# OvO1111/JointImageGeneration

Hardware: AMD Instinct MI355X
Metric: sampled voxels/sec @50 DDIM steps, 128^3 mask + 512^2x256 CT (higher is better)
Workload: dtype bf16; 1 GPU; C5 full GuideGen volume per GPU: CCDM 128^3 K=14 250 steps -> LDM 256 slices x (cond-encode + 50 DDIM @4x64x64 + AE decode 512^2); volumes_per_gpu=1, ccdm_steps=250, ddim_steps=50, slices=256, parallelism=replicas x1 (one volume per GPU, no collective), weights=random-init (seed recipe)

## Files before the change

include/guidegen_hip.h:

```cpp
#ifndef GUIDEGEN_HIP_H
#define GUIDEGEN_HIP_H

#include <stdint.h>

#ifdef __cplusplus
extern "C" {
#endif

typedef enum {
    GG_OK = 0,
    GG_ERR_BAD_SHAPE = -1,
    GG_ERR_BAD_DTYPE = -2,
    GG_ERR_UNSUPPORTED = -3,
    GG_ERR_WORKSPACE_TOO_SMALL = -4,
    GG_ERR_HIP = -5
} gg_status;

typedef enum { GG_BF16 = 0, GG_F32 = 1 } gg_dtype;

const char *gg_last_error(void);
int gg_version(void);

typedef struct {
    int32_t N, D, H, W;
// ... 30 lines not shown
    int32_t pro_c_logical;
    const int64_t *pro_acc1;
    const int64_t *pro_acc2;
    const float *pro_gamma;
    const float *pro_beta;
    float pro_eps;
    int32_t skip_C1, skip_C2;
    int32_t reserved_tail;
    const void *skip_src1;
    const void *skip_src2;
    const void *skip_weight;
    const int32_t *post_xt;
    int32_t *post_labels_out;
    const float *post_scalars;
    const float *post_E;
    uint64_t post_philox_seed;
    const int64_t *post_philox_offset_dev;
    void *post_onehot_out;
    int64_t post_onehot_stride;
    int32_t post_draw;
    int32_t reserved_tail2;
    const uint64_t *post_philox_seeds;
    int64_t post_rows_per_sample;
} gg_conv_desc;

int64_t gg_conv_packed_weight_bytes(int32_t Cout, int32_t Cin_pad, int32_t ntaps);
int gg_conv_pack_weight(const float *w_f32, int32_t Cout, int32_t Cin, int32_t Cin_pad, int32_t ntaps,
                        void *packed_bf16, void *stream);
int64_t gg_conv_workspace_bytes(const gg_conv_desc *desc);
int gg_conv_fuses_prologue(const gg_conv_desc *desc);
int gg_conv_fuses_posterior(const gg_conv_desc *desc);
int gg_conv_runs_halo_tile(const gg_conv_desc *desc);
int gg_conv_runs_tile(const gg_conv_desc *desc);
int gg_conv_runs_halo_split(const gg_conv_desc *desc);
int gg_conv_runs_tile_s2(const gg_conv_desc *desc);
int gg_conv_emits_stats(const gg_conv_desc *desc);
int gg_conv_prologue_from_acc(const gg_conv_desc *desc);
int gg_conv_fuses_skip(const gg_conv_desc *desc);
int gg_conv_fuses_ddim(const gg_conv_desc *desc);
int gg_conv_forward(const gg_conv_desc *desc, void *stream);

int64_t gg_groupnorm_workspace_bytes(int32_t N, int64_t S, int32_t C);
int gg_groupnorm_stats(const void *src1, int32_t C1, const void *src2, int32_t C2, int32_t N, int64_t S,
                       int32_t C_logical, const float *gamma, const float *beta, float eps,
                       float *scale_out, float *shift_out, void *workspace, int64_t workspace_bytes, void *stream);
int gg_groupnorm_apply(const void *src1, int32_t C1, const void *src2, int32_t C2, int32_t N, int64_t S,
                       const float *scale, const float *shift, int32_t act, void *out, void *stream);
int gg_groupnorm_fused_supported(int64_t S, int32_t C1, int32_t C2, int32_t C_logical);
int gg_groupnorm_fused(const void *src1, int32_t C1, const void *src2, int32_t C2, int32_t N, int64_t S, int32_t C_logical,
                       const float *gamma, const float *beta, float eps, int32_t act, void *out, void *stream);
int gg_groupnorm_apply_acc(const void *src1, int32_t C1, const int64_t *acc1, const void *src2, int32_t C2, const int64_t *acc2,
                           int32_t N, int64_t S, int32_t C_logical, const float *gamma, const float *beta, float eps,
                           int32_t act, void *out, void *stream);

int gg_groupnorm_scale_shift_acc(const int64_t *acc1, int32_t stripes1, int32_t C1, const int64_t *acc2, int32_t stripes2, int32_t C2,
                                 int32_t N, int64_t S, int32_t C_logical, const float *gamma, const float *beta, float eps,
                                 float *scale_out, float *shift_out, void *stream);

int gg_resample2x(const void *src, int32_t dtype, int32_t N, int32_t D, int32_t H, int32_t W, int32_t C_pad, int32_t C_logical,
                  int32_t resample_d, int32_t mode, const float *scale, const float *shift, int32_t act, void *dst, void *stream);
int gg_film_fold(float *scale, float *shift, int32_t coef_stride, int32_t N, int32_t C, const float *film, int64_t film_stride, void *stream);

typedef struct {
    int32_t N, heads, head_dim;
    int32_t Tq, Tkv;
    int64_t ldq, hsq, ldk, hsk, ldv, hsv, ldo, hso;
    float scale;
    int32_t reserved;
    const void *q, *k, *v;
    void *out;
    void *workspace;
    int64_t workspace_bytes;
} gg_attention_desc;
int gg_attention_forward(const gg_attention_desc *desc, void *stream);
int64_t gg_attention_workspace_bytes(const gg_attention_desc *desc);
int gg_attention_plan(const gg_attention_desc *desc, int32_t plan[4]);
int gg_attention_forward_kvlen(const gg_attention_desc *desc, const int32_t *kv_len, void *stream);

// ... 158 lines not shown
```

jointimagegeneration_amd/csrc/gg_conv.h:

```cpp
#pragma once
#include "gg_common.h"

struct ConvParams {
    int N, D, H, W, C1, C2, Cout, Cout_pad;
    int kd, kh, kw, stride, pad, upsample;
    int Do, Ho, Wo, out_dtype, prologue_act;
    int path_hint;
    int nchunk1, nchunk, ntaps;
    long long M;
    long long bias_stride;
    const bf16_t *src1, *src2, *weight, *residual;
    const float *bias, *gn_scale, *gn_shift;
    void *out;
    float *ws;
    int splitk;
    long long *gn_acc;
    float *ddim_x, *ddim_pred_x0;
    const float *ddim_scalars;
    bf16_t *ddim_unet_in;
    long long ddim_unet_in_stride;
    unsigned mg_osp, mg_ohw, mg_wo;
    int epi_geglu;
    const long long *pro_acc1, *pro_acc2;
    const float *pro_gamma, *pro_beta;
// ... 41 lines not shown

__device__ __forceinline__ float gg_row16_sum(float x)
{
    x += __builtin_bit_cast(float, __builtin_amdgcn_mov_dpp(__builtin_bit_cast(int, x), 0xB1, 0xF, 0xF, true));
    x += __builtin_bit_cast(float, __builtin_amdgcn_mov_dpp(__builtin_bit_cast(int, x), 0x4E, 0xF, 0xF, true));
    x += __builtin_bit_cast(float, __builtin_amdgcn_mov_dpp(__builtin_bit_cast(int, x), 0x141, 0xF, 0xF, true));
    x += __builtin_bit_cast(float, __builtin_amdgcn_mov_dpp(__builtin_bit_cast(int, x), 0x140, 0xF, 0xF, true));
    return x;
}

__device__ __forceinline__ f32x4 gg_conv_epi_value(f32x4 acc, bool has_bias, f32x4 bv, bool has_res, bf16x4 res, int co, int Cout)
{
    f32x4 v = acc;
    if (has_bias) v += bv;
    if (has_res) {
#pragma unroll
        for (int j = 0; j < 4; ++j) v[j] += (float)res[j];
    }
#pragma unroll
    for (int j = 0; j < 4; ++j)
        if (co + j >= Cout) v[j] = 0.f;
    return v;
}
__device__ __forceinline__ bf16x4 gg_conv_epi_bf16(f32x4 v)
{
    bf16x4 ob;
#pragma unroll
    for (int j = 0; j < 4; ++j) ob[j] = (bf16_t)v[j];
    return ob;
}

int gg_conv_tile_try(const ConvParams &p, hipStream_t stream);
int gg_conv_tile_family(const ConvParams &p);
bool gg_conv_tile_s2_family(const ConvParams &p);
int gg_conv_tile_s2_launch(const ConvParams &p, hipStream_t stream);
bool gg_conv_halo_split_box_fits(const ConvParams &p);
int gg_conv_halo_split_launch(const ConvParams &p, hipStream_t stream);
```

jointimagegeneration_amd/csrc/gg_conv.hip:

```cpp
#include "gg_norm.h"
#include <stdlib.h>

template <int NT, int PF, int PRO>
__global__ __launch_bounds__(256) void conv_gather_kernel(const ConvParams p)
{
    constexpr int BM = 128;
    constexpr int XBYTES = BM * 64;
    constexpr int WBYTES = NT * 32 * 64;
    constexpr int STAGE = XBYTES + WBYTES;
    constexpr int WITER = (NT * 128 + 255) / 256;
    __shared__ __attribute__((aligned(16))) char smem[2 * STAGE];

    const int tid = threadIdx.x;
    const int lane = tid & 63;
    const int wave = tid >> 6;
    const long long m0 = (long long)blockIdx.x * BM;
    const int g0 = blockIdx.y * NT;

    const int xq = tid & 3;
    int bn[2], bd[2], bh[2], bw[2];
    bool rv[2];
    const bf16_t *rb1[2], *rb2[2];
    const unsigned osp = (unsigned)(p.Do * p.Ho * p.Wo);
    const unsigned ohw = (unsigned)(p.Ho * p.Wo);
// ... 767 lines not shown
    if (!GG_HALO_SPLIT || !gg_hint_is_production(p.path_hint) || p.path_hint == GG_CONV_HINT_NO_HALO_SPLIT) return 0;
    if (p.kd != 3 || p.kh != 3 || p.kw != 3 || p.stride != 1 || p.pad != 1 || p.upsample || p.prologue_act) return 0;
    if (d->epilogue_geglu || d->post_xt || d->ddim_x || d->skip_C1) return 0;
    if (halo_try_dry(p) || box_try_dry(p) || !gg_conv_halo_split_box_fits(p)) return 0;
    if (gg_conv_tiny_plan(p.M, p.Cout_pad, p.ntaps * p.nchunk, p.prologue_act) || plan_gather5(p.M, p.C1, p.C2, p.Cout_pad, p.ntaps)) return 0;
    const GatherPlan pl = plan_gather(p.M, p.Cout_pad, p.ntaps * p.nchunk);
    return (pl.NT == 1 && pl.splitk >= 2 && p.nchunk % pl.splitk == 0) ? pl.splitk : 0;
}

extern "C" int gg_conv_runs_halo_split(const gg_conv_desc *d)
{
    if (!desc_channels_ok(d)) return 0;
    ConvParams p;
    fill_params(d, p);
    return plan_halo_split(d, p);
}

static bool plan_tile_s2(const gg_conv_desc *d, const ConvParams &p)
{
    if (!gg_conv_tile_s2_family(p) || halo_try_dry(p) || box_try_dry(p)) return false;
    if (p.path_hint == GG_CONV_HINT_TILE_S2) return true;
    if (gg_conv_tiny_plan(p.M, p.Cout_pad, p.ntaps * p.nchunk, p.prologue_act) || plan_gather5(p.M, p.C1, p.C2, p.Cout_pad, p.ntaps)) return false;
    return plan_gather(p.M, p.Cout_pad, p.ntaps * p.nchunk).splitk == 1;
}

extern "C" int gg_conv_runs_tile_s2(const gg_conv_desc *d)
{
    if (!desc_channels_ok(d)) return 0;
    ConvParams p;
    fill_params(d, p);
    return plan_tile_s2(d, p) ? 1 : 0;
}

#ifdef GG_EXP_WPREFETCH
__global__ __launch_bounds__(256) void exp_wprefetch_kernel(const u32x4 *w, long long n16, unsigned *sink)
{
    unsigned a = 0;
    if (n16 <= (3 << 20) / 16 * 1) {
        for (long long i = (long long)(blockIdx.x >> 3) * 256 + threadIdx.x; i < n16; i += 32 * 256) { const u32x4 v = w[i]; a ^= v[0] ^ v[1] ^ v[2] ^ v[3]; }
    } else
    for (long long i = (long long)blockIdx.x * 256 + threadIdx.x; i < n16; i += 256 * 256) { const u32x4 v = w[i]; a ^= v[0] ^ v[1] ^ v[2] ^ v[3]; }
    if (a == 0x12345679u) sink[0] = a;
}
#endif
extern "C" int gg_conv_forward(const gg_conv_desc *d, void *stream_)
{
    hipStream_t stream = (hipStream_t)stream_;
    if (!d) GG_FAIL(GG_ERR_BAD_SHAPE, "conv: null desc");
    if (d->C1 <= 0 || d->C1 % 32 || d->C2 % 32 || d->C2 < 0) GG_FAIL(GG_ERR_BAD_SHAPE, "conv: C1/C2 must be multiples of 32 (got %d, %d)", d->C1, d->C2);
    if (d->Cout_pad % 32 || d->Cout > d->Cout_pad || d->Cout <= 0) GG_FAIL(GG_ERR_BAD_SHAPE, "conv: bad Cout/Cout_pad %d/%d", d->Cout, d->Cout_pad);
    auto okk = [](int k) { return k == 1 || k == 3; };
    if (!okk(d->kd) || !okk(d->kh) || !okk(d->kw)) GG_FAIL(GG_ERR_UNSUPPORTED, "conv: kernel extent must be 1 or 3");
    if (d->stride != 1 && d->stride != 2) GG_FAIL(GG_ERR_UNSUPPORTED, "conv: stride must be 1 or 2");
    if (d->upsample && d->stride != 1) GG_FAIL(GG_ERR_UNSUPPORTED, "conv: upsample with stride");
    if (d->out_dtype != GG_BF16 && d->out_dtype != GG_F32) GG_FAIL(GG_ERR_BAD_DTYPE, "conv: out dtype");
    if (!d->src1 || !d->weight || (!d->out && !d->post_xt) || (d->C2 && !d->src2)) GG_FAIL(GG_ERR_BAD_SHAPE, "conv: null pointer");
    if (d->post_xt) {
        if (!gg_conv_fuses_posterior(d)) GG_FAIL(GG_ERR_UNSUPPORTED, "conv: this shape cannot run the fused CCDM reverse step (gg_conv_fuses_posterior)");
        if (!d->post_labels_out || !d->post_scalars) GG_FAIL(GG_ERR_BAD_SHAPE, "conv: fused CCDM reverse step needs labels_out and scalars");
        if (d->post_onehot_out && (d->post_onehot_stride < d->Cout || (d->post_onehot_stride & 1) || ((uintptr_t)d->post_onehot_out & 3)))
            GG_FAIL(GG_ERR_BAD_SHAPE, "conv: fused CCDM reverse step: one-hot rows must be 4-byte aligned (even stride >= K)");
        if (d->post_philox_seeds && d->post_rows_per_sample != (int64_t)d->Do * d->Ho * d->Wo)
            GG_FAIL(GG_ERR_BAD_SHAPE, "conv: fused CCDM reverse step: post_rows_per_sample %lld must be Do*Ho*Wo = %lld",
                    (long long)d->post_rows_per_sample, (long long)d->Do * d->Ho * d->Wo);
    }
    const bool pro_acc = d->prologue_act && !d->gn_scale && !d->gn_shift && d->pro_acc1;
// ... 28 lines not shown
            d->ddim_x || d->Cout % 32 || d->bias_stride)
            GG_FAIL(GG_ERR_UNSUPPORTED, "conv: the GEGLU epilogue needs a 1x1 conv, bf16 output, Cout = 2*inner with inner %% 16 == 0, a shared bias, no residual / gn_acc / ddim");
        return launch_gather_nt(plan_gather(p.M, p.Cout_pad, p.ntaps * p.nchunk).NT, p, stream);
    }
#ifdef GG_EXP_WPREFETCH
    {
        const long long wbytes = (long long)(p.Cout_pad / 32) * p.ntaps * p.nchunk * 2048;
        hipLaunchKernelGGL(exp_wprefetch_kernel, dim3(256), dim3(256), 0, stream, (const u32x4 *)p.weight, wbytes >> 4, (unsigned *)d->out);
    }
#endif
#ifdef GG_H3_STAMPS
    if (d->path_hint == GG_HALO_HINT_TEAM && d->workspace) p.ws = (float *)d->workspace;
#endif
    int rc = gg_conv_halo_try(p, stream);
#ifdef GG_H3_STAMPS
    p.ws = nullptr;
#endif
    if (rc != GG_ERR_UNSUPPORTED) return rc;
    if (d->post_xt) GG_FAIL(GG_ERR_UNSUPPORTED, "conv: the halo-tile kernel did not take this shape, and no other kernel runs the fused CCDM reverse step");
#ifdef GG_BOX_STAMPS
    if (d->path_hint == 98) p.ws = (float *)d->workspace;
#endif
    rc = gg_conv_box_try(p, stream);
#ifdef GG_BOX_STAMPS
    p.ws = nullptr;
#endif
    if (rc != GG_ERR_UNSUPPORTED) return rc;

    rc = gg_conv_tile_try(p, stream);
    if (rc != GG_ERR_UNSUPPORTED) return rc;

    if (plan_tile_s2(d, p)) return gg_conv_tile_s2_launch(p, stream);

    if (int hs = plan_halo_split(d, p)) {
        if ((rc = take_splitk_workspace(d, p, hs)) != GG_OK) return rc;
        if ((rc = gg_conv_halo_split_launch(p, stream)) != GG_OK) return rc;
        return launch_splitk_reduce(p, stream, true);
    }

    if (int tsk = gg_conv_tiny_plan(p.M, p.Cout_pad, p.ntaps * p.nchunk, p.prologue_act)) {
        if ((rc = take_splitk_workspace(d, p, tsk)) != GG_OK) return rc;
        rc = gg_conv_tiny_launch(p, stream);
        if (rc != GG_OK || tsk == 1) return rc;
        return launch_splitk_reduce(p, stream, false);
    }

    if (int s5 = plan_gather5(p.M, p.C1, p.C2, p.Cout_pad, p.ntaps)) {
        if ((rc = take_splitk_workspace(d, p, s5)) != GG_OK) return rc;
        dim3 grid((unsigned)((p.M + 63) / 64), (unsigned)(p.Cout_pad / 32), (unsigned)s5);
        if (p.prologue_act && (((long long)p.Do * p.Ho * p.Wo) % 64 || p.C1 + p.C2 > 2560))
            GG_FAIL(GG_ERR_UNSUPPORTED, "conv: fused prologue on the 160-step kernel needs Do*Ho*Wo %% 64 == 0 and C <= 2560");
        if (p.prologue_act) hipLaunchKernelGGL(conv_gather5_kernel<1>, grid, dim3(256), 0, stream, p);
        else hipLaunchKernelGGL(conv_gather5_kernel<0>, grid, dim3(256), 0, stream, p);
        GG_CHECK_LAUNCH();
        return s5 > 1 ? launch_splitk_reduce(p, stream, true) : GG_OK;
    }

    GatherPlan pl = plan_gather(p.M, p.Cout_pad, p.ntaps * p.nchunk);
    if ((rc = take_splitk_workspace(d, p, pl.splitk)) != GG_OK) return rc;
    return launch_gather_nt(pl.NT, p, stream);
}
```

jointimagegeneration_amd/csrc/gg_norm.hip:

```cpp
#include "gg_norm.h"

__global__ __launch_bounds__(256) void gn_partial_kernel(const bf16_t *__restrict__ s1, int C1,
                                                         const bf16_t *__restrict__ s2, int C2, long long S,
                                                         long long rows_per_block, float *__restrict__ part)
{
    const int C = C1 + C2;
    const int P = C >> 3;
    const int rpi = blockDim.x / P;
    const int tid = threadIdx.x;
    const int piece = tid % P, rsub = tid / P;
    const int n = blockIdx.y;
    const long long r0 = (long long)blockIdx.x * rows_per_block;
    long long r1 = r0 + rows_per_block;
    if (r1 > S) r1 = S;
    float sum[8], sq[8];
#pragma unroll
    for (int j = 0; j < 8; ++j) sum[j] = sq[j] = 0.f;
    if (rsub < rpi) {
        const int c0 = piece * 8;
        const bool second = c0 >= C1;
        const bf16_t *base = second ? s2 + (long long)n * S * C2 + (c0 - C1) : s1 + (long long)n * S * C1 + c0;
        const int Cs = second ? C2 : C1;
        for (long long r = r0 + rsub; r < r1; r += rpi) {
            bf16x8 v = *reinterpret_cast<const bf16x8 *>(base + r * Cs);
#pragma unroll
            for (int j = 0; j < 8; ++j) {
                float f = (float)v[j];
                sum[j] += f;
                sq[j] += f * f;
            }
        }
    }
    extern __shared__ float red[];
#pragma unroll
    for (int j = 0; j < 8; ++j) {
        red[tid * 16 + j] = sum[j];
        red[tid * 16 + 8 + j] = sq[j];
    }
    __syncthreads();
    if (tid < P) {
        float a[16];
#pragma unroll
        for (int j = 0; j < 16; ++j) a[j] = 0.f;
        for (int k = 0; k < rpi; ++k)
#pragma unroll
            for (int j = 0; j < 16; ++j) a[j] += red[(k * P + tid) * 16 + j];
        float *dst = part + (((long long)n * gridDim.x + blockIdx.x) * C + tid * 8) * 2;
#pragma unroll
        for (int j = 0; j < 8; ++j) {
            dst[2 * j] = a[j];
            dst[2 * j + 1] = a[8 + j];
        }
    }
}

__global__ __launch_bounds__(256) void gn_finalize_kernel(const float *__restrict__ part, int nblk, int C, int C_logical,
                                                          long long S, const float *__restrict__ gamma,
                                                          const float *__restrict__ beta, float eps,
                                                          float *__restrict__ scale, float *__restrict__ shift)
{
    const int n = blockIdx.y, g = blockIdx.x;
    const int cpg = C_logical / 32;
    const int tid = threadIdx.x;
    __shared__ double ra[256], rb[256];
    double a = 0.0, b = 0.0;
    const int total = nblk * cpg;
    for (int i0 = tid; i0 < total; i0 += 1024) {
        float2 v[4];
#pragma unroll
        for (int u = 0; u < 4; ++u) {
            const int i = i0 + 256 * u;
            v[u] = float2{0.f, 0.f};
            if (i < total) {
                const int k = i / cpg, j = i - k * cpg;
                v[u] = *reinterpret_cast<const float2 *>(part + (((long long)n * nblk + k) * C + g * cpg + j) * 2);
            }
        }
#pragma unroll
        for (int u = 0; u < 4; ++u) { a += (double)v[u].x; b += (double)v[u].y; }
    }
    ra[tid] = a;
    rb[tid] = b;
    __syncthreads();
    for (int s = 128; s > 0; s >>= 1) {
        if (tid < s) { ra[tid] += ra[tid + s]; rb[tid] += rb[tid + s]; }
        __syncthreads();
    }
    float fmean, frstd;
    gn_moments_ieee(ra[0], rb[0], (double)S * cpg, eps, fmean, frstd);
    if (tid < cpg) {
        const int c = g * cpg + tid;
        const float sc = gn_scale(frstd, gamma[c]);
        scale[(long long)n * C + c] = sc;
        shift[(long long)n * C + c] = gn_shift(beta[c], fmean, sc);
    }
    if (g == 0) gn_zero_pad_lanes(scale, shift, n, C, C_logical, tid);
}

__global__ __launch_bounds__(256) void gn_stats_small_kernel(const bf16_t *__restrict__ s1, int C1, const bf16_t *__restrict__ s2,
                                                             int C2, long long S, int C_logical, const float *__restrict__ gamma,
                                                             const float *__restrict__ beta, float eps, float *__restrict__ scale,
                                                             float *__restrict__ shift)
{
    s1 = gg_pin(s1); C1 = gg_pin(C1); s2 = gg_pin(s2); C2 = gg_pin(C2); S = gg_pin(S); C_logical = gg_pin(C_logical);
    gamma = gg_pin(gamma); beta = gg_pin(beta); eps = gg_pin(eps); scale = gg_pin(scale); shift = gg_pin(shift);
    const int C = C1 + C2;
    const int n = blockIdx.y, g = blockIdx.x, tid = threadIdx.x;
    const int cpg = C_logical / 32;
    const bf16_t *b1 = s1 + (long long)n * S * C1;
    const bf16_t *b2 = s2 ? s2 + (long long)n * S * C2 : nullptr;
    float a = 0.f, b = 0.f;
    float gmm = 0.f, bta = 0.f;
    if (tid < cpg) { gmm = gamma[g * cpg + tid]; bta = beta[g * cpg + tid]; }
    const int c_lo = g * cpg, c_hi = c_lo + cpg;
    const int p_lo = c_lo >> 3, p_hi = (c_hi - 1) >> 3;
    const int np = p_hi - p_lo + 1;
    const int work = (int)S * np;
    const float rnp = __builtin_amdgcn_rcpf((float)np);
    for (int i = tid; i < work; i += 256) {
        const int r = gg_div_small(i, rnp);
        const int c0 = (p_lo + (i - r * np)) * 8;
        const bf16x8 v = *reinterpret_cast<const bf16x8 *>(gn_piece_ptr(b1, C1, b2, C2, (long long)r, c0));
#pragma unroll
        for (int j = 0; j < 8; ++j) {
            const int c = c0 + j;
            const float f = (c >= c_lo && c < c_hi) ? (float)v[j] : 0.f;
            a += f;
            b += f * f;
        }
// ... 122 lines not shown
{
    return (C1 > 0 && C1 % 32 == 0 && C2 >= 0 && C2 % 32 == 0 && gn_fused_small_ok(S, C1, C2, C_logical)) ? 1 : 0;
}

extern "C" int gg_groupnorm_fused(const void *src1, int32_t C1, const void *src2, int32_t C2, int32_t N, int64_t S, int32_t C_logical,
                                  const float *gamma, const float *beta, float eps, int32_t act, void *out, void *stream_)
{
    hipStream_t stream = (hipStream_t)stream_;
    GN_CHECK("groupnorm_fused", C1, C2, 0, nullptr, false, src1 && (!C2 || src2) && gamma && beta && out && N > 0 && S > 0, "null pointer / empty");
    if (!gn_fused_small_ok(S, C1, C2, C_logical)) GG_FAIL(GG_ERR_UNSUPPORTED, "groupnorm_fused: tensor too large for the single-launch path (gg_groupnorm_fused_supported)");
    hipLaunchKernelGGL(gn_fused_small_kernel, dim3(32, N), dim3(256), 0, stream, (const bf16_t *)src1, C1, (const bf16_t *)src2, C2,
                       (long long)S, gamma, beta, eps, act, (bf16_t *)out);
    GG_CHECK_LAUNCH();
    return GG_OK;
}

extern "C" int64_t gg_groupnorm_workspace_bytes(int32_t N, int64_t S, int32_t C)
{
    (void)S;
    return (int64_t)N * 1024 * C * 2 * 4;
}

static int gn_nblk(int N, long long S, int C)
{
    long long want = (2048 + N - 1) / N;
    long long maxb = (S + 63) / 64;
    long long nb = want < maxb ? want : maxb;
    if (nb < 1) nb = 1;
    if (nb > 1024) nb = 1024;
    (void)C;
    return (int)nb;
}

extern "C" int gg_groupnorm_stats(const void *src1, int32_t C1, const void *src2, int32_t C2, int32_t N, int64_t S,
                                  int32_t C_logical, const float *gamma, const float *beta, float eps, float *scale_out,
                                  float *shift_out, void *workspace, int64_t workspace_bytes, void *stream_)
{
    hipStream_t stream = (hipStream_t)stream_;
    const int C = C1 + C2;
    GN_CHECK("groupnorm", C1, C2, C_logical, GN_LOGICAL_TEXT, true, src1 && (!C2 || src2) && gamma && beta && scale_out && shift_out && workspace, "null pointer");
    if ((long long)S * C <= (1 << 19)) {
        hipLaunchKernelGGL(gn_stats_small_kernel, dim3(32, N), dim3(256), 0, stream, (const bf16_t *)src1, C1, (const bf16_t *)src2, C2,
                           (long long)S, C_logical, gamma, beta, eps, scale_out, shift_out);
        GG_CHECK_LAUNCH();
        return GG_OK;
    }
    const int nblk = gn_nblk(N, S, C);
    if ((int64_t)N * nblk * C * 8 > workspace_bytes) GG_FAIL(GG_ERR_WORKSPACE_TOO_SMALL, "groupnorm: workspace %lld < %lld", (long long)workspace_bytes, (long long)N * nblk * C * 8);
    const long long rpb = (S + nblk - 1) / nblk;
    hipLaunchKernelGGL(gn_partial_kernel, dim3(nblk, N), dim3(256), 256 * 16 * sizeof(float), stream, (const bf16_t *)src1, C1,
                       (const bf16_t *)src2, C2, (long long)S, rpb, (float *)workspace);
    GG_CHECK_LAUNCH();
    hipLaunchKernelGGL(gn_finalize_kernel, dim3(32, N), dim3(256), 0, stream, (const float *)workspace, nblk, C, C_logical,
                       (long long)S, gamma, beta, eps, scale_out, shift_out);
    GG_CHECK_LAUNCH();
    return GG_OK;
}

__global__ __launch_bounds__(256) void gn_apply_kernel(const bf16_t *__restrict__ s1, int C1, const bf16_t *__restrict__ s2,
                                                       int C2, long long S, long long total_pieces,
                                                       const float *__restrict__ scale, const float *__restrict__ shift,
                                                       int act, bf16_t *__restrict__ out, unsigned pmagic, int N)
{
    s1 = gg_pin(s1); C1 = gg_pin(C1); s2 = gg_pin(s2); C2 = gg_pin(C2); S = gg_pin(S); total_pieces = gg_pin(total_pieces);
    scale = gg_pin(scale); shift = gg_pin(shift); act = gg_pin(act); out = gg_pin(out); pmagic = gg_pin(pmagic); N = gg_pin(N);
    const int C = C1 + C2;
    const int P = C >> 3;
    for (long long i = (long long)blockIdx.x * 256 + threadIdx.x; i < total_pieces; i += (long long)gridDim.x * 256) {
        long long row = gg_fastdiv(i, P, pmagic);
        int piece = (int)(i - row * P);
        int c0 = piece * 8;
        int n = N == 1 ? 0 : (int)(row / S);
        const bf16_t *src = gn_piece_ptr(s1, C1, s2, C2, row, c0);
        bf16x8 v = *reinterpret_cast<const bf16x8 *>(src);
        const float *sc = scale + (long long)n * C + c0;
        const float *sh = shift + (long long)n * C + c0;
        f32x4 a0 = *reinterpret_cast<const f32x4 *>(sc), a1 = *reinterpret_cast<const f32x4 *>(sc + 4);
        f32x4 b0 = *reinterpret_cast<const f32x4 *>(sh), b1 = *reinterpret_cast<const f32x4 *>(sh + 4);
        *reinterpret_cast<bf16x8 *>(out + row * C + c0) = gn_affine8(v, a0, a1, b0, b1, act);
    }
}

extern "C" int gg_groupnorm_apply(const void *src1, int32_t C1, const void *src2, int32_t C2, int32_t N, int64_t S,
                                  const float *scale, const float *shift, int32_t act, void *out, void *stream_)
{
    hipStream_t stream = (hipStream_t)stream_;
    GN_CHECK("groupnorm_apply", C1, C2, 0, nullptr, false, src1 && (!C2 || src2) && scale && shift && out, "null pointer");
    long long total = (long long)N * S * ((C1 + C2) / 8);
    const unsigned blocks = gg_blocks256(total, 8192);
// ... 392 lines not shown
```

jointimagegeneration_amd/ops.py:

```python
from __future__ import annotations

import ctypes as C
from dataclasses import dataclass
from typing import Optional, Sequence, Tuple

import torch

from . import _lib
from ._lib import GG_BF16, GG_F32, AttentionDesc, ConvDesc, call, check


def _stream() -> int:
    return torch.cuda.current_stream().cuda_stream


def _ptr(t: Optional[torch.Tensor]) -> Optional[int]:
    return None if t is None else t.data_ptr()


def require_gpu(t: torch.Tensor, what: str) -> None:
    if not t.is_cuda:
        raise RuntimeError(f"{what}: tensor is on {t.device}; the GuideGen engine runs on MI355X only "
                           "(no CPU fallback; the CPU restatement lives in oracle/ and is test infrastructure)")

# ... 326 lines not shown
        oh = post.get("onehot_out")
        d.post_xt, d.post_labels_out, d.post_scalars = post["xt"].data_ptr(), post["labels_out"].data_ptr(), post["scalars"].data_ptr()
        d.post_E = _ptr(post.get("E"))
        d.post_philox_seed = int(post.get("philox_seed", 0))
        d.post_philox_offset_dev = _ptr(post.get("philox_offset"))
        d.post_draw = 1 if post.get("draw", True) else 0
        d.post_onehot_out, d.post_onehot_stride = _ptr(oh), (oh.shape[-1] if oh is not None else 0)
        seeds = post.get("philox_seeds")
        if seeds is not None:
            d.post_philox_seeds, d.post_rows_per_sample = _seeds_ptr(seeds, N), Do * Ho * Wo
        fused_post = True
    call("gg_conv_forward", C.byref(d), _stream())
    return CL(out, cout // 2 if geglu else cout, acc=acc, fused_ddim=fused, fused_post=fused_post)


def _gn_sources(src1: CL, src2: Optional[CL], padded_first: str = "raise"):
    if src2 is not None and src1.C != src1.Cpad and padded_first != "ignore":
        if padded_first == "none":
            return None
        raise RuntimeError("two-source GroupNorm needs an unpadded first source")
    if src2 is None:
        return src1.N, src1.S, src1.Cpad, 0, src1.C, None
    return src1.N, src1.S, src1.Cpad, src2.Cpad, src1.C + src2.C, src2.t.data_ptr()


def _gn_out(src1: CL, Ct: int, dtype=torch.bfloat16) -> torch.Tensor:
    return torch.empty(tuple(src1.t.shape[:4]) + (Ct,), dtype=dtype, device=src1.t.device)


def _gn_tables(src1: CL, N: int, Ct: int):
    return tuple(torch.empty((N, Ct), dtype=torch.float32, device=src1.t.device) for _ in range(2))


def groupnorm_stats(src1: CL, gamma: torch.Tensor, beta: torch.Tensor, eps: float, src2: Optional[CL] = None):
    lib = _lib.load()
    N, S, C1, C2, c_log, p2 = _gn_sources(src1, src2)
    ws_bytes = lib.gg_groupnorm_workspace_bytes(N, S, C1 + C2)
    ws = torch.empty(ws_bytes // 4, dtype=torch.float32, device=src1.t.device)
    scale, shift = _gn_tables(src1, N, C1 + C2)
    call("gg_groupnorm_stats", src1.t.data_ptr(), C1, p2, C2, N, S, c_log, gamma.data_ptr(), beta.data_ptr(), eps, scale.data_ptr(),
         shift.data_ptr(), ws.data_ptr(), ws_bytes, _stream())
    return scale, shift


def groupnorm_apply(src1: CL, scale: torch.Tensor, shift: torch.Tensor, act: bool, src2: Optional[CL] = None) -> CL:
    N, S, C1, C2, c_log, p2 = _gn_sources(src1, src2, "ignore")
    out = _gn_out(src1, C1 + C2)
    call("gg_groupnorm_apply", src1.t.data_ptr(), C1, p2, C2, N, S, scale.data_ptr(), shift.data_ptr(), 1 if act else 0, out.data_ptr(), _stream())
    return CL(out, c_log)


def groupnorm_fused_ok(src1: CL, src2: Optional[CL] = None) -> bool:
    hdr = None if is_f32(src1.t) else _gn_sources(src1, src2, "none")
    return hdr is not None and bool(_lib.load().gg_groupnorm_fused_supported(hdr[1], hdr[2], hdr[3], hdr[4]))


def groupnorm_fused(src1: CL, gamma: torch.Tensor, beta: torch.Tensor, eps: float, act: bool, src2: Optional[CL] = None) -> CL:
    N, S, C1, C2, c_log, p2 = _gn_sources(src1, src2, "ignore")
    out = _gn_out(src1, C1 + C2)
    call("gg_groupnorm_fused", src1.t.data_ptr(), C1, p2, C2, N, S, c_log, gamma.data_ptr(), beta.data_ptr(), eps, 1 if act else 0, out.data_ptr(),
         _stream())
    return CL(out, c_log)


def groupnorm_f32(src1: CL, gamma: torch.Tensor, beta: torch.Tensor, eps: float, act: bool, src2: Optional[CL] = None) -> CL:
    N, S, C1, C2, c_log, p2 = _gn_sources(src1, src2)
    out = _gn_out(src1, C1 + C2, torch.float32)
    ws = torch.empty(64 * N, dtype=torch.float32, device=src1.t.device)
    call("gg_groupnorm_f32", src1.t.data_ptr(), C1, p2, C2, N, S, c_log, gamma.data_ptr(), beta.data_ptr(), eps, 1 if act else 0, out.data_ptr(),
         ws.data_ptr(), _stream())
    return CL(out, c_log)


def groupnorm_f32_film(src: CL, gamma: torch.Tensor, beta: torch.Tensor, eps: float, film: torch.Tensor, act: bool) -> CL:
# ... 1059 lines not shown
```

Baseline: 831,400 voxels/s.

## Add row-wise 1x1 conv kernel and single-launch GroupNorm stats path

Adds a dedicated 1x1 convolution kernel for small-M bf16 convs that keeps the whole weight slice in LDS and double-buffers activation loads, chosen ahead of the halo-split and gather paths when no split-K is planned. It also adds a one-launch GroupNorm statistics kernel that computes per-block partials and finalizes them in the same kernel for mid-sized tensors, replacing the partial+finalize two-launch sequence. Both target launch overhead and inefficiency on small LDM-sized tensors, at the cost of lower parallelism per group (32xN blocks) and a new selection path that could pick a slower kernel for some shapes.

```diff
diff --git a/include/guidegen_hip.h b/include/guidegen_hip.h
--- a/include/guidegen_hip.h
+++ b/include/guidegen_hip.h
@@ -86,6 +86,7 @@
 int gg_conv_fuses_posterior(const gg_conv_desc *desc);
 int gg_conv_runs_halo_tile(const gg_conv_desc *desc);
 int gg_conv_runs_tile(const gg_conv_desc *desc);
+int gg_conv_runs_row1x1(const gg_conv_desc *desc);
 int gg_conv_runs_halo_split(const gg_conv_desc *desc);
 int gg_conv_runs_tile_s2(const gg_conv_desc *desc);
 int gg_conv_emits_stats(const gg_conv_desc *desc);
@@ -98,6 +99,9 @@
 int gg_groupnorm_stats(const void *src1, int32_t C1, const void *src2, int32_t C2, int32_t N, int64_t S,
                        int32_t C_logical, const float *gamma, const float *beta, float eps,
                        float *scale_out, float *shift_out, void *workspace, int64_t workspace_bytes, void *stream);
+int gg_groupnorm_stats_path(const void *src1, int32_t C1, const void *src2, int32_t C2, int32_t N, int64_t S,
+                            int32_t C_logical, const float *gamma, const float *beta, float eps,
+                            float *scale_out, float *shift_out, void *workspace, int64_t workspace_bytes, int32_t path, void *stream);
 int gg_groupnorm_apply(const void *src1, int32_t C1, const void *src2, int32_t C2, int32_t N, int64_t S,
                        const float *scale, const float *shift, int32_t act, void *out, void *stream);
 int gg_groupnorm_fused_supported(int64_t S, int32_t C1, int32_t C2, int32_t C_logical);
diff --git a/jointimagegeneration_amd/csrc/gg_conv.h b/jointimagegeneration_amd/csrc/gg_conv.h
--- a/jointimagegeneration_amd/csrc/gg_conv.h
+++ b/jointimagegeneration_amd/csrc/gg_conv.h
@@ -97,6 +97,8 @@
 
 int gg_conv_tile_try(const ConvParams &p, hipStream_t stream);
 int gg_conv_tile_family(const ConvParams &p);
+bool gg_conv_row1x1_family(const ConvParams &p);
+int gg_conv_row1x1_launch(const ConvParams &p, hipStream_t stream);
 bool gg_conv_tile_s2_family(const ConvParams &p);
 int gg_conv_tile_s2_launch(const ConvParams &p, hipStream_t stream);
 bool gg_conv_halo_split_box_fits(const ConvParams &p);
diff --git a/jointimagegeneration_amd/csrc/gg_conv.hip b/jointimagegeneration_amd/csrc/gg_conv.hip
--- a/jointimagegeneration_amd/csrc/gg_conv.hip
+++ b/jointimagegeneration_amd/csrc/gg_conv.hip
@@ -823,6 +823,21 @@
     return plan_tile_s2(d, p) ? 1 : 0;
 }
 
+static bool plan_row1x1(const ConvParams &p)
+{
+    if (!gg_conv_row1x1_family(p) || halo_try_dry(p) || box_try_dry(p) || gg_conv_tile_family(p)) return false;
+    if (gg_conv_tiny_plan(p.M, p.Cout_pad, p.ntaps * p.nchunk, p.prologue_act) || plan_gather5(p.M, p.C1, p.C2, p.Cout_pad, p.ntaps)) return false;
+    return plan_gather(p.M, p.Cout_pad, p.ntaps * p.nchunk).splitk == 1;
+}
+
+extern "C" int gg_conv_runs_row1x1(const gg_conv_desc *d)
+{
+    if (!desc_channels_ok(d) || d->epilogue_geglu) return 0;
+    ConvParams p;
+    fill_params(d, p);
+    return plan_row1x1(p) ? 1 : 0;
+}
+
 #ifdef GG_EXP_WPREFETCH
 __global__ __launch_bounds__(256) void exp_wprefetch_kernel(const u32x4 *w, long long n16, unsigned *sink)
 {
@@ -917,6 +932,8 @@
 
     if (plan_tile_s2(d, p)) return gg_conv_tile_s2_launch(p, stream);
 
+    if (plan_row1x1(p)) return gg_conv_row1x1_launch(p, stream);
+
     if (int hs = plan_halo_split(d, p)) {
         if ((rc = take_splitk_workspace(d, p, hs)) != GG_OK) return rc;
         if ((rc = gg_conv_halo_split_launch(p, stream)) != GG_OK) return rc;
diff --git a/jointimagegeneration_amd/csrc/gg_conv_row1x1.hip b/jointimagegeneration_amd/csrc/gg_conv_row1x1.hip
--- /dev/null
+++ b/jointimagegeneration_amd/csrc/gg_conv_row1x1.hip
@@ -0,0 +1,133 @@
+#include "gg_conv.h"
+
+#ifndef GG_ROW1X1
+#define GG_ROW1X1 1
+#endif
+
+#define GG_ROW1X1_MAX_M 8192
+
+#define ROW1X1_XB 8
+#define ROW1X1_LDS_MAX 65536
+
+template <int NG>
+__global__ __launch_bounds__(256) void conv_row1x1_kernel(const ConvParams p)
+{
+    constexpr int XB = ROW1X1_XB, CT = 2 * NG;
+    extern __shared__ __attribute__((aligned(16))) char smem[];
+    const int tid = threadIdx.x, lane = tid & 63;
+    const int wave = __builtin_amdgcn_readfirstlane(tid >> 6);
+    const int fr = lane & 15, fq = lane >> 4;
+    const long long m0 = (long long)blockIdx.x * 64;
+    const int g0 = blockIdx.y * NG;
+    const int nch = p.nchunk, nch1 = p.nchunk1;
+    const unsigned osp = (unsigned)(p.Do * p.Ho * p.Wo);
+    const long long m = m0 + wave * 16 + fr;
+    const bool mvalid = m < p.M;
+
+    f32x4 bv[CT];
+    bf16x4 resv[CT];
+#pragma unroll
+    for (int ct = 0; ct < CT; ++ct) {
+        const int co = g0 * 32 + ct * 16 + fq * 4;
+        bv[ct] = f32x4{0.f, 0.f, 0.f, 0.f};
+        resv[ct] = bf16x4{};
+        if (mvalid) {
+            if (p.bias) bv[ct] = *reinterpret_cast<const f32x4 *>(p.bias + (long long)((unsigned)m / osp) * p.bias_stride + co);
+            if (p.residual) resv[ct] = *reinterpret_cast<const bf16x4 *>(p.residual + m * p.Cout_pad + co);
+        }
+    }
+
+    const bf16_t *b1 = p.src1 + m * p.C1 + fq * 8;
+    const bf16_t *b2 = p.src2 ? p.src2 + m * p.C2 + fq * 8 : nullptr;
+    auto load_x = [&](u32x4 (&x)[XB], int c0) {
+#pragma unroll
+        for (int j = 0; j < XB; ++j) {
+            const int c = c0 + j;
+            u32x4 v = {0u, 0u, 0u, 0u};
+            if (c < nch && mvalid) v = *reinterpret_cast<const u32x4 *>(c < nch1 ? b1 + c * 32 : b2 + (c - nch1) * 32);
+            x[j] = v;
+        }
+    };
+    u32x4 xa[XB], xb[XB];
+    load_x(xa, 0);
+    load_x(xb, XB);
+
+    {
+        const bf16_t *wsrc = p.weight + (((long long)g0 * nch) << 10);
+        const int pieces = NG * nch * 128;
+        for (int i0 = tid; i0 < pieces; i0 += 8 * 256) {
+            u32x4 w[8];
+#pragma unroll
+            for (int u = 0; u < 8; ++u)
+                if (i0 + 256 * u < pieces) w[u] = *reinterpret_cast<const u32x4 *>(wsrc + (long long)(i0 + 256 * u) * 8);
+#pragma unroll
+            for (int u = 0; u < 8; ++u)
+                if (i0 + 256 * u < pieces) *reinterpret_cast<u32x4 *>(smem + (i0 + 256 * u) * 16) = w[u];
+        }
+    }
+    __syncthreads();
+
+    f32x4 acc[CT];
+#pragma unroll
+    for (int ct = 0; ct < CT; ++ct) acc[ct] = f32x4{0.f, 0.f, 0.f, 0.f};
+    auto compute = [&](const u32x4 (&x)[XB], int c0) {
+#pragma unroll
+        for (int j = 0; j < XB; ++j) {
+            const int c = c0 + j;
+            if (c < nch) {
+                const bf16x8 xf = __builtin_bit_cast(bf16x8, x[j]);
+#pragma unroll
+                for (int ct = 0; ct < CT; ++ct) {
+                    const int r = (ct & 1) * 16 + fr;
+                    const bf16x8 wf = *reinterpret_cast<const bf16x8 *>(smem + ((ct >> 1) * nch + c) * 2048 + r * 64 + swz64(r, fq) * 16);
+                    acc[ct] = __builtin_amdgcn_mfma_f32_16x16x32_bf16(wf, xf, acc[ct], 0, 0, 0);
+                }
+            }
+        }
+    };
+    for (int c0 = 0; c0 < nch; c0 += 2 * XB) {
+        compute(xa, c0);
+        if (c0 + 2 * XB < nch) load_x(xa, c0 + 2 * XB);
+        if (c0 + XB < nch) {
+            compute(xb, c0 + XB);
+            if (c0 + 3 * XB < nch) load_x(xb, c0 + 3 * XB);
+        }
+    }
+
+#pragma unroll
+    for (int ct = 0; ct < CT; ++ct) {
+        const int co = g0 * 32 + ct * 16 + fq * 4;
+        if (!mvalid) continue;
+        const f32x4 v = gg_conv_epi_value(acc[ct], p.bias != nullptr, bv[ct], p.residual != nullptr, resv[ct], co, p.Cout);
+        *reinterpret_cast<bf16x4 *>((bf16_t *)p.out + m * p.Cout_pad + co) = gg_conv_epi_bf16(v);
+    }
+}
+
+static int row1x1_ng(const ConvParams &p)
+{
+    const int G = p.Cout_pad / 32;
+    const long long mb = (p.M + 63) / 64;
+    return (G % 2 == 0 && 2 * p.nchunk * 2048 <= ROW1X1_LDS_MAX && mb * (G / 2) >= 256) ? 2 : 1;
+}
+
+bool gg_conv_row1x1_family(const ConvParams &p)
+{
+    if (!GG_ROW1X1 || p.path_hint == GG_CONV_HINT_GATHER) return false;
+    if (p.kd != 1 || p.kh != 1 || p.kw != 1 || p.stride != 1 || p.upsample) return false;
+    if (p.Do != p.D || p.Ho != p.H || p.Wo != p.W) return false;
+    if (p.prologue_act || p.out_dtype != GG_BF16 || p.epi_geglu || p.post_xt || p.ddim_x || p.skip_C1) return false;
+    if (p.nchunk * 2048 > ROW1X1_LDS_MAX) return false;
+    if (p.M > GG_ROW1X1_MAX_M) return false;
+    return true;
+}
+
+int gg_conv_row1x1_launch(const ConvParams &p, hipStream_t stream)
+{
+    const int ng = row1x1_ng(p);
+    const dim3 grid((unsigned)((p.M + 63) / 64), (unsigned)(p.Cout_pad / (32 * ng)));
+    const size_t lds = (size_t)ng * p.nchunk * 2048;
+    if (ng == 2) hipLaunchKernelGGL(conv_row1x1_kernel<2>, grid, dim3(256), lds, stream, p);
+    else hipLaunchKernelGGL(conv_row1x1_kernel<1>, grid, dim3(256), lds, stream, p);
+    GG_CHECK_LAUNCH();
+    return GG_OK;
+}
diff --git a/jointimagegeneration_amd/csrc/gg_norm.hip b/jointimagegeneration_amd/csrc/gg_norm.hip
--- a/jointimagegeneration_amd/csrc/gg_norm.hip
+++ b/jointimagegeneration_amd/csrc/gg_norm.hip
@@ -54,33 +54,34 @@
     }
 }
 
-__global__ __launch_bounds__(256) void gn_finalize_kernel(const float *__restrict__ part, int nblk, int C, int C_logical,
-                                                          long long S, const float *__restrict__ gamma,
-                                                          const float *__restrict__ beta, float eps,
-                                                          float *__restrict__ scale, float *__restrict__ shift)
-{
-    const int n = blockIdx.y, g = blockIdx.x;
+template <class Pair>
+__device__ __forceinline__ void gn_finalize_group(Pair pair, int nblk, int n, int g, int C, int C_logical, long long S,
+                                                  const float *__restrict__ gamma, const float *__restrict__ beta, float eps,
+                                                  float *__restrict__ scale, float *__restrict__ shift)
+{
     const int cpg = C_logical / 32;
     const int tid = threadIdx.x;
     __shared__ double ra[256], rb[256];
     double a = 0.0, b = 0.0;
     const int total = nblk * cpg;
-    for (int i0 = tid; i0 < total; i0 += 1024) {
-        float2 v[4];
-#pragma unroll
-        for (int u = 0; u < 4; ++u) {
-            const int i = i0 + 256 * u;
-            v[u] = float2{0.f, 0.f};
-            if (i < total) {
-                const int k = i / cpg, j = i - k * cpg;
-                v[u] = *reinterpret_cast<const float2 *>(part + (((long long)n * nblk + k) * C + g * cpg + j) * 2);
-            }
-        }
-#pragma unroll
-        for (int u = 0; u < 4; ++u) { a += (double)v[u].x; b += (double)v[u].y; }
-    }
-    ra[tid] = a;
-    rb[tid] = b;
+    if (tid < 256) {
+        for (int i0 = tid; i0 < total; i0 += 1024) {
+            float2 v[4];
+#pragma unroll
+            for (int u = 0; u < 4; ++u) {
+                const int i = i0 + 256 * u;
+                v[u] = float2{0.f, 0.f};
+                if (i < total) {
+                    const int k = i / cpg, j = i - k * cpg;
+                    v[u] = pair(k, j);
+                }
+            }
+#pragma unroll
+            for (int u = 0; u < 4; ++u) { a += (double)v[u].x; b += (double)v[u].y; }
+        }
+        ra[tid] = a;
+        rb[tid] = b;
+    }
     __syncthreads();
     for (int s = 128; s > 0; s >>= 1) {
         if (tid < s) { ra[tid] += ra[tid + s]; rb[tid] += rb[tid + s]; }
@@ -94,7 +95,90 @@
         scale[(long long)n * C + c] = sc;
         shift[(long long)n * C + c] = gn_shift(beta[c], fmean, sc);
     }
-    if (g == 0) gn_zero_pad_lanes(scale, shift, n, C, C_logical, tid);
+    if (g == 0 && tid < 256) gn_zero_pad_lanes(scale, shift, n, C, C_logical, tid);
+}
+
+__global__ __launch_bounds__(256) void gn_finalize_kernel(const float *__restrict__ part, int nblk, int C, int C_logical,
+                                                          long long S, const float *__restrict__ gamma,
+                                                          const float *__restrict__ beta, float eps,
+                                                          float *__restrict__ scale, float *__restrict__ shift)
+{
+    const int n = blockIdx.y, g = blockIdx.x;
+    const int cpg = C_logical / 32;
+    gn_finalize_group([=](int k, int j) { return *reinterpret_cast<const float2 *>(part + (((long long)n * nblk + k) * C + g * cpg + j) * 2); },
+                      nblk, n, g, C, C_logical, S, gamma, beta, eps, scale, shift);
+}
+
+#define GG_GN_GROUP_THREADS 1024
+#define GG_GN_GROUP_KC 64
+#define GG_GN_GROUP_ROWS 8
+__global__ __launch_bounds__(GG_GN_GROUP_THREADS) void gn_stats_group_kernel(const bf16_t *__restrict__ s1, int C1, const bf16_t *__restrict__ s2,
+                                                                             int C2, long long S, long long rows_per_block, int nblk,
+                                                                             int C_logical, const float *__restrict__ gamma,
+                                                                             const float *__restrict__ beta, float eps,
+                                                                             float *__restrict__ scale, float *__restrict__ shift)
+{
+    const int C = C1 + C2;
+    const int n = blockIdx.y, g = blockIdx.x, tid = threadIdx.x;
+    const int cpg = C_logical / 32;
+    const int rpi = 256 / (C >> 3);
+    const int c_lo = g * cpg, c_hi = c_lo + cpg;
+    const int p_lo = c_lo >> 3;
+    const int np = ((c_hi - 1) >> 3) - p_lo + 1;
+    __shared__ float2 slot[GG_GN_GROUP_KC * 64];
+    extern __shared__ float2 part[];
+    const int per_k = np * rpi;
+    for (int k0 = 0; k0 < nblk; k0 += GG_GN_GROUP_KC) {
+        const int kc = nblk - k0 < GG_GN_GROUP_KC ? nblk - k0 : GG_GN_GROUP_KC;
+        for (int t = tid; t < kc * per_k; t += GG_GN_GROUP_THREADS) {
+            const int kk = t / per_k, q = t - kk * per_k;
+            const int rsub = q / np, c0 = (p_lo + (q - rsub * np)) * 8;
+            const long long r0 = (long long)(k0 + kk) * rows_per_block;
+            long long r1 = r0 + rows_per_block;
+            if (r1 > S) r1 = S;
+            const bool second = c0 >= C1;
+            const bf16_t *base = second ? s2 + (long long)n * S * C2 + (c0 - C1) : s1 + (long long)n * S * C1 + c0;
+            const int Cs = second ? C2 : C1;
+            float sum[8], sq[8];
+#pragma unroll
+            for (int j = 0; j < 8; ++j) sum[j] = sq[j] = 0.f;
+            for (long long r = r0 + rsub; r < r1; r += GG_GN_GROUP_ROWS * rpi) {
+                u32x4 v[GG_GN_GROUP_ROWS];
+#pragma unroll
+                for (int u = 0; u < GG_GN_GROUP_ROWS; ++u) {
+                    const long long ru = r + (long long)u * rpi;
+                    v[u] = u32x4{0u, 0u, 0u, 0u};
+                    if (ru < r1) v[u] = *reinterpret_cast<const u32x4 *>(base + ru * Cs);
+                }
+#pragma unroll
+                for (int u = 0; u < GG_GN_GROUP_ROWS; ++u)
+#pragma unroll
+                    for (int j = 0; j < 8; ++j) {
+                        float f = (float)__builtin_bit_cast(bf16x8, v[u])[j];
+                        sum[j] += f;
+                        sq[j] += f * f;
+                    }
+            }
+#pragma unroll
+            for (int j = 0; j < 8; ++j) {
+                const int cl = c0 + j - c_lo;
+                if (cl >= 0 && cl < cpg) slot[(kk * rpi + rsub) * cpg + cl] = float2{sum[j], sq[j]};
+            }
+        }
+        __syncthreads();
+        for (int i = tid; i < kc * cpg; i += GG_GN_GROUP_THREADS) {
+            const int kk = i / cpg, cl = i - kk * cpg;
+            float a = 0.f, b = 0.f;
+            for (int k = 0; k < rpi; ++k) {
+                const float2 v = slot[(kk * rpi + k) * cpg + cl];
+                a += v.x;
+                b += v.y;
+            }
+            part[(k0 + kk) * cpg + cl] = float2{a, b};
+        }
+        __syncthreads();
+    }
+    gn_finalize_group([=](int k, int j) { return part[k * cpg + j]; }, nblk, n, g, C, C_logical, S, gamma, beta, eps, scale, shift);
 }
 
 __global__ __launch_bounds__(256) void gn_stats_small_kernel(const bf16_t *__restrict__ s1, int C1, const bf16_t *__restrict__ s2,
@@ -283,22 +367,43 @@
     return (int)nb;
 }
 
-extern "C" int gg_groupnorm_stats(const void *src1, int32_t C1, const void *src2, int32_t C2, int32_t N, int64_t S,
-                                  int32_t C_logical, const float *gamma, const float *beta, float eps, float *scale_out,
-                                  float *shift_out, void *workspace, int64_t workspace_bytes, void *stream_)
+#ifndef GG_GN_GROUP
+#define GG_GN_GROUP 1
+#endif
+#ifndef GG_GN_GROUP_MAX
+#define GG_GN_GROUP_MAX (4096LL * 576)
+#endif
+#define GG_GN_PATH_AUTO 0
+#define GG_GN_PATH_TWO_LAUNCH 1
+#define GG_GN_PATH_GROUP 2
+#define GG_GN_GROUP_PART_BYTES (24 * 1024)
+
+extern "C" int gg_groupnorm_stats_path(const void *src1, int32_t C1, const void *src2, int32_t C2, int32_t N, int64_t S,
+                                       int32_t C_logical, const float *gamma, const float *beta, float eps, float *scale_out,
+                                       float *shift_out, void *workspace, int64_t workspace_bytes, int32_t path, void *stream_)
 {
     hipStream_t stream = (hipStream_t)stream_;
     const int C = C1 + C2;
     GN_CHECK("groupnorm", C1, C2, C_logical, GN_LOGICAL_TEXT, true, src1 && (!C2 || src2) && gamma && beta && scale_out && shift_out && workspace, "null pointer");
-    if ((long long)S * C <= (1 << 19)) {
+    if (path != GG_GN_PATH_AUTO && path != GG_GN_PATH_TWO_LAUNCH && path != GG_GN_PATH_GROUP) GG_FAIL(GG_ERR_BAD_SHAPE, "groupnorm: unknown path %d", path);
+    if (path == GG_GN_PATH_AUTO && (long long)S * C <= (1 << 19)) {
         hipLaunchKernelGGL(gn_stats_small_kernel, dim3(32, N), dim3(256), 0, stream, (const bf16_t *)src1, C1, (const bf16_t *)src2, C2,
                            (long long)S, C_logical, gamma, beta, eps, scale_out, shift_out);
         GG_CHECK_LAUNCH();
         return GG_OK;
     }
     const int nblk = gn_nblk(N, S, C);
+    const long long rpb = (S + nblk - 1) / nblk;
+    const size_t part_bytes = (size_t)nblk * (C_logical / 32) * sizeof(float2);
+    const bool fits = part_bytes <= GG_GN_GROUP_PART_BYTES;
+    if (path == GG_GN_PATH_GROUP && !fits) GG_FAIL(GG_ERR_UNSUPPORTED, "groupnorm: %d partial blocks x %d channels do not fit the one-launch path", nblk, C_logical / 32);
+    if (path == GG_GN_PATH_GROUP || (path == GG_GN_PATH_AUTO && GG_GN_GROUP && fits && (long long)S * C <= GG_GN_GROUP_MAX)) {
+        hipLaunchKernelGGL(gn_stats_group_kernel, dim3(32, N), dim3(GG_GN_GROUP_THREADS), part_bytes, stream, (const bf16_t *)src1, C1,
+                           (const bf16_t *)src2, C2, (long long)S, rpb, nblk, C_logical, gamma, beta, eps, scale_out, shift_out);
+        GG_CHECK_LAUNCH();
+        return GG_OK;
+    }
     if ((int64_t)N * nblk * C * 8 > workspace_bytes) GG_FAIL(GG_ERR_WORKSPACE_TOO_SMALL, "groupnorm: workspace %lld < %lld", (long long)workspace_bytes, (long long)N * nblk * C * 8);
-    const long long rpb = (S + nblk - 1) / nblk;
     hipLaunchKernelGGL(gn_partial_kernel, dim3(nblk, N), dim3(256), 256 * 16 * sizeof(float), stream, (const bf16_t *)src1, C1,
                        (const bf16_t *)src2, C2, (long long)S, rpb, (float *)workspace);
     GG_CHECK_LAUNCH();
@@ -306,6 +411,14 @@
                        (long long)S, gamma, beta, eps, scale_out, shift_out);
     GG_CHECK_LAUNCH();
     return GG_OK;
+}
+
+extern "C" int gg_groupnorm_stats(const void *src1, int32_t C1, const void *src2, int32_t C2, int32_t N, int64_t S,
+                                  int32_t C_logical, const float *gamma, const float *beta, float eps, float *scale_out,
+                                  float *shift_out, void *workspace, int64_t workspace_bytes, void *stream_)
+{
+    return gg_groupnorm_stats_path(src1, C1, src2, C2, N, S, C_logical, gamma, beta, eps, scale_out, shift_out, workspace, workspace_bytes,
+                                   GG_GN_PATH_AUTO, stream_);
 }
 
 __global__ __launch_bounds__(256) void gn_apply_kernel(const bf16_t *__restrict__ s1, int C1, const bf16_t *__restrict__ s2,
diff --git a/jointimagegeneration_amd/ops.py b/jointimagegeneration_amd/ops.py
--- a/jointimagegeneration_amd/ops.py
+++ b/jointimagegeneration_amd/ops.py
@@ -382,14 +382,20 @@
     return tuple(torch.empty((N, Ct), dtype=torch.float32, device=src1.t.device) for _ in range(2))
 
 
-def groupnorm_stats(src1: CL, gamma: torch.Tensor, beta: torch.Tensor, eps: float, src2: Optional[CL] = None):
+GN_PATH_AUTO, GN_PATH_TWO_LAUNCH, GN_PATH_GROUP = 0, 1, 2
+
+
+def groupnorm_stats(src1: CL, gamma: torch.Tensor, beta: torch.Tensor, eps: float, src2: Optional[CL] = None, path: Optional[int] = None):
     lib = _lib.load()
     N, S, C1, C2, c_log, p2 = _gn_sources(src1, src2)
     ws_bytes = lib.gg_groupnorm_workspace_bytes(N, S, C1 + C2)
     ws = torch.empty(ws_bytes // 4, dtype=torch.float32, device=src1.t.device)
     scale, shift = _gn_tables(src1, N, C1 + C2)
-    call("gg_groupnorm_stats", src1.t.data_ptr(), C1, p2, C2, N, S, c_log, gamma.data_ptr(), beta.data_ptr(), eps, scale.data_ptr(),
-         shift.data_ptr(), ws.data_ptr(), ws_bytes, _stream())
+    args = (src1.t.data_ptr(), C1, p2, C2, N, S, c_log, gamma.data_ptr(), beta.data_ptr(), eps, scale.data_ptr(), shift.data_ptr(), ws.data_ptr(), ws_bytes)
+    if path is None:
+        call("gg_groupnorm_stats", *args, _stream())
+    else:
+        call("gg_groupnorm_stats_path", *args, path, _stream())
     return scale, shift
 
 
```

Result: no change. 827,700 voxels/s (-0.4%).
